# MaxInGaussian/SCFGP

Hardware: AMD Instinct MI355X
Metric: NLML+grad evals/sec (higher is better)
Workload: dtype f32

## Files before the change

scfgp_amd/csrc/kernels_kstage.hip:

```cpp
#include "kernels.h"
#include "tile_engine.h"

#ifndef SCFGP_KSTAGE_BK
#define SCFGP_KSTAGE_BK 16
#endif
#ifndef SCFGP_KSTAGE_WGM
#define SCFGP_KSTAGE_WGM 2
#define SCFGP_KSTAGE_WGN 2
#endif
typedef TileCfg<double, 64, 64, SCFGP_KSTAGE_BK, SCFGP_KSTAGE_WGM, SCFGP_KSTAGE_WGN> KCfg;
#define SMEM_DECL extern __shared__ __attribute__((aligned(16))) char smem_raw[]

struct GemmArgs {
    const double* A; const double* B; double* C;
    int64_t lda, ldb, ldc;
    int M, N, K;
    double alpha, beta;
    int tri;
    int kskip;
};

template <bool TRA, bool TRB>
__device__ __forceinline__ void gemm64_body(const GemmArgs& a, int tm, int tn, double* smem) {
    typedef KCfg Cfg;
    if (tm * Cfg::BM >= a.M || tn * Cfg::BN >= a.N) return;
    if (a.tri && tn > tm) return;
    const int k0 = a.kskip == 1 ? (tm > tn ? tm : tn) * Cfg::BM : (a.kskip == 2 ? tn * Cfg::BN : (a.kskip == 4 ? tm * Cfg::BM : 0));
    const int k1 = a.kskip == 3 && (tm + 1) * Cfg::BM < a.K ? (tm + 1) * Cfg::BM : a.K;
    const int nkt = (k1 - k0) / Cfg::BK;
    v4d acc[Cfg::TM][Cfg::TN];
    acc_zero<Cfg>(acc);
    if (TRA) {
        TrLoader<double, double, Cfg::BM, Cfg::BK, Cfg::LDA, Cfg::THREADS, false, false, 3> la(a.A + (int64_t)tm * Cfg::BM * a.lda + k0, a.lda, threadIdx.x);
        if (TRB) {
            TrLoader<double, double, Cfg::BN, Cfg::BK, Cfg::LDB, Cfg::THREADS, false, false, 3> lb(a.B + (int64_t)tn * Cfg::BN * a.ldb + k0, a.ldb, threadIdx.x);
            tile_mainloop_deep3<Cfg>(la, lb, nkt, acc, smem);
        } else {
            NatLoader<double, double, Cfg::BN, Cfg::BK, Cfg::LDB, Cfg::THREADS, false, false, false, 3> lb(a.B + (int64_t)k0 * a.ldb + tn * Cfg::BN, a.ldb, threadIdx.x);
            tile_mainloop_deep3<Cfg>(la, lb, nkt, acc, smem);
        }
    } else {
        NatLoader<double, double, Cfg::BM, Cfg::BK, Cfg::LDA, Cfg::THREADS, false, false, false, 3> la(a.A + (int64_t)k0 * a.lda + tm * Cfg::BM, a.lda, threadIdx.x);
        if (TRB) {
            TrLoader<double, double, Cfg::BN, Cfg::BK, Cfg::LDB, Cfg::THREADS, false, false, 3> lb(a.B + (int64_t)tn * Cfg::BN * a.ldb + k0, a.ldb, threadIdx.x);
            tile_mainloop_deep3<Cfg>(la, lb, nkt, acc, smem);
        } else {
            NatLoader<double, double, Cfg::BN, Cfg::BK, Cfg::LDB, Cfg::THREADS, false, false, false, 3> lb(a.B + (int64_t)k0 * a.ldb + tn * Cfg::BN, a.ldb, threadIdx.x);
            tile_mainloop_deep3<Cfg>(la, lb, nkt, acc, smem);
        }
    }
    AccCoord<Cfg> co;
#pragma unroll
    for (int t1 = 0; t1 < Cfg::TM; ++t1)
#pragma unroll
        for (int r = 0; r < Cfg::MTr::NACC; ++r) {
            double* c = a.C + (int64_t)(tm * Cfg::BM + co.row(t1, r)) * a.ldc + tn * Cfg::BN;
#pragma unroll
            for (int t2 = 0; t2 < Cfg::TN; ++t2) {
                const double v = a.alpha * acc[t1][t2][r];
                c[co.col(t2)] = a.beta == 0.0 ? v : v + a.beta * c[co.col(t2)];
                if (a.tri == 2 && tm != tn) a.C[(int64_t)(tn * Cfg::BN + co.col(t2)) * a.ldc + tm * Cfg::BM + co.row(t1, r)] = v;
            }
        }
}

template <bool TRA, bool TRB>
__global__ __launch_bounds__(KCfg::THREADS) void gemm64_kernel(GemmArgs a) {
    SMEM_DECL;
    gemm64_body<TRA, TRB>(a, blockIdx.y, blockIdx.x, reinterpret_cast<double*>(smem_raw));
}

template <bool TRA, bool TRB>
static void gemm64(const GemmArgs& a, hipStream_t st) {
    if (a.M <= 0 || a.N <= 0) return;
    allow_big_lds(gemm64_kernel<TRA, TRB>, KCfg::LDS_BYTES);
    hipLaunchKernelGGL((gemm64_kernel<TRA, TRB>), dim3(a.N / KCfg::BN, a.M / KCfg::BM), dim3(KCfg::THREADS), KCfg::LDS_BYTES, st, a);
}

__device__ __forceinline__ double lane_bcast(double x, int lane) {
    const int lo = __builtin_amdgcn_readlane(__double2loint(x), lane), hi = __builtin_amdgcn_readlane(__double2hiint(x), lane);
    return __hiloint2double(hi, lo);
}
template <int NS>
__device__ __forceinline__ v4d mfma_tile(const double* pa, int lda, const double* pb, int ldbk, int ldbj, v4d acc, double sign) {
    const int lane = threadIdx.x & 63, i = lane & 15, q = lane >> 4;
#pragma unroll
    for (int s = 0; s < NS; ++s)
        acc = __builtin_amdgcn_mfma_f64_16x16x4f64(sign * pa[i * lda + 4 * s + q], pb[(4 * s + q) * ldbk + i * ldbj], acc, 0, 0, 0);
    return acc;
}
template <int LD>
__device__ __forceinline__ void block_xwt(const double* sX, const double* sW, v4d (&acc)[4]) {
    const int wave = threadIdx.x >> 6, lane = threadIdx.x & 63, i = lane & 15, q = lane >> 4;
#pragma unroll
    for (int b = 0; b < 4; ++b) acc[b] = v4d{0, 0, 0, 0};
#pragma unroll
    for (int s = 0; s < 16; ++s) {
        const double x = sX[(16 * wave + i) * LD + 4 * s + q];
#pragma unroll
        for (int b = s / 4; b < 4; ++b)
            acc[b] = __builtin_amdgcn_mfma_f64_16x16x4f64(x, sW[(16 * b + i) * LD + 4 * s + q], acc[b], 0, 0, 0);
    }
}
template <typename P>
__device__ __forceinline__ void block_store(P* dst, int64_t pitch, const v4d (&acc)[4]) {
    const int wave = threadIdx.x >> 6, lane = threadIdx.x & 63, ci = lane & 15, cq = lane >> 4;
#pragma unroll
    for (int b = 0; b < 4; ++b)
#pragma unroll
        for (int r = 0; r < 4; ++r) dst[(int64_t)(16 * wave + cq + 4 * r) * pitch + 16 * b + ci] = acc[b][r];
}
__device__ __forceinline__ void block_load(const double* src, int64_t pitch, v4d (&acc)[4]) {
    const int wave = threadIdx.x >> 6, lane = threadIdx.x & 63, ci = lane & 15, cq = lane >> 4;
#pragma unroll
    for (int b = 0; b < 4; ++b)
#pragma unroll
        for (int r = 0; r < 4; ++r) acc[b][r] = src[(int64_t)(16 * wave + cq + 4 * r) * pitch + 16 * b + ci];
}
template <int LD>
__device__ __forceinline__ void block_sub_pqt(const double* sP, const double* sQ, v4d (&acc)[4]) {
    const int wave = threadIdx.x >> 6, lane = threadIdx.x & 63, i = lane & 15, q = lane >> 4;
#pragma unroll
    for (int s = 0; s < 16; ++s) {
        const double x = -sP[(16 * wave + i) * LD + 4 * s + q];
#pragma unroll
        for (int b = 0; b < 4; ++b)
            acc[b] = __builtin_amdgcn_mfma_f64_16x16x4f64(x, sQ[(16 * b + i) * LD + 4 * s + q], acc[b], 0, 0, 0);
    }
}
template <int LD>
__device__ __forceinline__ void block_add_pqt(const double* sP, const double* sQ, v4d (&acc)[4]) {
    const int wave = threadIdx.x >> 6, lane = threadIdx.x & 63, i = lane & 15, q = lane >> 4;
#pragma unroll
    for (int s = 0; s < 16; ++s) {
        const double x = sP[(16 * wave + i) * LD + 4 * s + q];
#pragma unroll
        for (int b = 0; b < 4; ++b)
            acc[b] = __builtin_amdgcn_mfma_f64_16x16x4f64(x, sQ[(16 * b + i) * LD + 4 * s + q], acc[b], 0, 0, 0);
    }
}
__device__ __forceinline__ void block_to_lds(const double* src, int64_t pitch, double* dst, int LD) {
    for (int e = threadIdx.x; e < 64 * 64; e += 256) dst[(e / 64) * LD + e % 64] = src[(int64_t)(e / 64) * pitch + e % 64];
}

#ifdef SCFGP_TRACE
__device__ unsigned long long g_ctrace[64][16];
#define CSTAMP(k) do { if (threadIdx.x == 0 && p < 64) g_ctrace[p][k] = __builtin_amdgcn_s_memrealtime(); } while (0)
int64_t chol_trace_read(void* host, int64_t max_bytes) {
    const int64_t n = max_bytes < (int64_t)sizeof(g_ctrace) ? max_bytes : (int64_t)sizeof(g_ctrace);
    return hipMemcpyFromSymbol(host, HIP_SYMBOL(g_ctrace), n) == hipSuccess ? n : -2;
}
#else
#define CSTAMP(k)
int64_t chol_trace_read(void*, int64_t) { return -1; }
#endif

__global__ __launch_bounds__(256) void chol_step_kernel(double* A, double* Lm, double* Li, double* Bm, int64_t ld, int p, int nb, int* flag) {
    constexpr int NB = 64, LD = NB + 1, PB = 16;
    __shared__ double sL[NB * LD];
    __shared__ double sI[NB * LD];
    __shared__ double sT[32 * 33];
    __shared__ double sD[NB];
    const int tid = threadIdx.x, lane = tid & 63, wave = tid >> 6;
    const int ci = lane & 15, cq = lane >> 4;
    v4d acc[4];
    if (blockIdx.x > 0) {
        const int q = p - 1, n = nb - p, T = n * (n + 1) / 2, U = p * n;
        int t = blockIdx.x - 1, i, j;
        bool b_tile = false;
        const auto tri_decode = [](int t, int& ti, int& tj) {
            ti = (int)((sqrtf(8.0f * t + 1.0f) - 1.0f) * 0.5f);
            while ((ti + 1) * (ti + 2) / 2 <= t) ++ti;
            while (ti * (ti + 1) / 2 > t) --ti;
            tj = t - ti * (ti + 1) / 2;
        };
        if (t < T) {
            int ti, tj; tri_decode(t, ti, tj);
            i = p + ti; j = p + tj;
            if (i == p && j == p) return;
        } else if (t < T + U) {
            t -= T; i = t / n; j = p + t % n;
        } else {
            tri_decode(t - T - U, i, j); b_tile = true;
        }
        const double* gw = Li + ((int64_t)q * ld + q) * NB;
        const double* gi = A + ((int64_t)i * ld + q) * NB;
        const double* gj = A + ((int64_t)j * ld + q) * NB;
        double* c = (b_tile ? Bm : A) + ((int64_t)i * ld + j) * NB;
        const bool unit_i = i == q, unit_j = j == q;
        const bool first_b = b_tile && i == q;
        v2d rw[8], ri[8], rj[8];
#pragma unroll
        for (int u = 0; u < 8; ++u) {
            const int e = (tid + u * 256) * 2;
            const int64_t o = (int64_t)(e / NB) * ld + e % NB;
            rw[u] = *reinterpret_cast<const v2d*>(gw + o);
            if (!unit_i) ri[u] = *reinterpret_cast<const v2d*>(gi + o);
            if (i != j && !unit_j) rj[u] = *reinterpret_cast<const v2d*>(gj + o);
        }
        v4d accc[4];
        if (!first_b) block_load(c, ld, accc);
        else {
#pragma unroll
            for (int b = 0; b < 4; ++b) accc[b] = v4d{0, 0, 0, 0};
        }
#pragma unroll
        for (int u = 0; u < 8; ++u) {
            const int e = (tid + u * 256) * 2, o = (e / NB) * LD + e % NB;
            sL[o] = rw[u][0]; sL[o + 1] = rw[u][1];
            if (!unit_i) { sI[o] = ri[u][0]; sI[o + 1] = ri[u][1]; }
        }
        __syncthreads();
        const auto w_transposed = [&](v4d (&a)[4]) {
#pragma unroll
            for (int b = 0; b < 4; ++b)
#pragma unroll
                for (int r = 0; r < 4; ++r) a[b][r] = sL[(16 * b + ci) * LD + 16 * wave + cq + 4 * r];
        };
        if (unit_i) w_transposed(acc);
        else block_xwt<LD>(sI, sL, acc);
        v4d accj[4];
        if (i != j) {
            if (unit_j) w_transposed(accj);
            else {
                __syncthreads();
#pragma unroll
                for (int u = 0; u < 8; ++u) {
                    const int e = (tid + u * 256) * 2, o = (e / NB) * LD + e % NB;
                    sI[o] = rj[u][0]; sI[o + 1] = rj[u][1];
                }
                __syncthreads();
                block_xwt<LD>(sI, sL, accj);
            }
            if (b_tile && unit_i) {
                double* d = Li + ((int64_t)q * ld + j) * NB;
#pragma unroll
                for (int b = 0; b < 4; ++b)
#pragma unroll
                    for (int r = 0; r < 4; ++r) d[(int64_t)(16 * b + ci) * ld + 16 * wave + cq + 4 * r] = accj[b][r];
            }
        }
        __syncthreads();
        block_store(sL, LD, acc);
        if (i != j) block_store(sI, LD, accj);
        __syncthreads();
        if (b_tile) {
            block_add_pqt<LD>(sL, i != j ? sI : sL, accc);
            block_store(c, ld, accc);
            if (i != j) {
                double* ct = Bm + ((int64_t)j * ld + i) * NB;
#pragma unroll
                for (int b = 0; b < 4; ++b)
#pragma unroll
                    for (int r = 0; r < 4; ++r) ct[(int64_t)(16 * b + ci) * ld + 16 * wave + cq + 4 * r] = accc[b][r];
            }
            return;
        }
        block_sub_pqt<LD>(sL, i != j ? sI : sL, accc);
        block_store(c, ld, accc);
        return;
    }
    if (p >= nb) return;
    CSTAMP(0);
    double* a = A + ((int64_t)p * ld + p) * NB;
    if (p > 0) {
        const double* gx = A + ((int64_t)p * ld + (p - 1)) * NB;
        const double* gw = Li + ((int64_t)(p - 1) * ld + (p - 1)) * NB;
        v2d rx[8], rw[8];
#pragma unroll
        for (int i = 0; i < 8; ++i) {
            const int e = (tid + i * 256) * 2;
            rx[i] = *reinterpret_cast<const v2d*>(gx + (int64_t)(e / NB) * ld + e % NB);
            rw[i] = *reinterpret_cast<const v2d*>(gw + (int64_t)(e / NB) * ld + e % NB);
        }
        v4d accd[4];
        block_load(a, ld, accd);
#pragma unroll
        for (int i = 0; i < 8; ++i) {
            const int e = (tid + i * 256) * 2, o = (e / NB) * LD + e % NB;
            sI[o] = rx[i][0]; sI[o + 1] = rx[i][1];
            sL[o] = rw[i][0]; sL[o + 1] = rw[i][1];
        }
        __syncthreads();
        CSTAMP(12);
        block_xwt<LD>(sI, sL, acc);
        __syncthreads();
        block_store(sI, LD, acc);
        __syncthreads();
        CSTAMP(13);
#pragma unroll
        for (int b = 0; b < 4; ++b) acc[b] = accd[b];
        CSTAMP(14);
        block_sub_pqt<LD>(sI, sI, acc);
        __syncthreads();
        CSTAMP(15);
        block_store(sL, LD, acc);
        for (int e = tid; e < NB * NB; e += 256) sI[(e / NB) * LD + e % NB] = 0.0;
    } else {
        for (int e = tid; e < NB * NB; e += 256) {
            sL[(e / NB) * LD + e % NB] = a[(int64_t)(e / NB) * ld + e % NB];
            sI[(e / NB) * LD + e % NB] = 0.0;
        }
    }
    double* lm = Lm + ((int64_t)p * ld + p) * NB;
    double* li = Li + ((int64_t)p * ld + p) * NB;
    bool bad = false;
    CSTAMP(1);
    const auto tile_update = [&](int r0, int c0, int pp) {
        v4d acc;
#pragma unroll
        for (int r = 0; r < 4; ++r) acc[r] = sL[(r0 + cq + 4 * r) * LD + c0 + ci];
        acc = mfma_tile<4>(sL + r0 * LD + pp, LD, sL + c0 * LD + pp, 1, LD, acc, -1.0);
#pragma unroll
        for (int r = 0; r < 4; ++r) sL[(r0 + cq + 4 * r) * LD + c0 + ci] = acc[r];
    };
    for (int pb = 0; pb < NB; pb += PB) {
        __syncthreads();
        const int nt = (NB - pb) / PB;
        if (wave == 0) {
            if (pb > 0)
                for (int ti = 0; ti < nt; ++ti) tile_update(pb + PB * ti, pb, pb - PB);
            const int row = pb + lane;
            double v[PB], invs[PB];
#pragma unroll
            for (int c = 0; c < PB; ++c) v[c] = row < NB ? sL[row * LD + pb + c] : 0.0;
#pragma unroll
            for (int j = 0; j < PB; ++j) {
                const double d = lane_bcast(v[j], j);
                bad |= !(d > 0.0);
                double inv = __builtin_amdgcn_rsq(d);
                inv = fma(0.5 * inv, fma(-d * inv, inv, 1.0), inv);
                inv = fma(0.5 * inv, fma(-d * inv, inv, 1.0), inv);
                invs[j] = inv;
                v[j] *= inv;
#pragma unroll
                for (int k = j + 1; k < PB; ++k) v[k] = fma(-v[j], lane_bcast(v[j], k), v[k]);
            }
#pragma unroll
            for (int c = 0; c < PB; ++c)
                if (row < NB) sL[row * LD + pb + c] = v[c];
            if (lane == 0) {
#pragma unroll
                for (int c = 0; c < PB; ++c) sD[pb + c] = invs[c];
            }
            CSTAMP(2 + pb / PB * 2);
            CSTAMP(3 + pb / PB * 2);
        } else if (pb > 0) {
            int t = 0;
            for (int tj = 1; tj < nt; ++tj)
                for (int ti = tj; ti < nt; ++ti, ++t)
                    if (t % 3 == wave - 1) tile_update(pb + PB * ti, pb + PB * tj, pb - PB);
        }
    }
    if (bad && tid == 0) *flag = 1;
    __syncthreads();
    if (tid < NB) {
        const int o = (tid / PB) * PB, c = tid % PB;
        double sres[PB];
#pragma unroll
        for (int r = 0; r < PB; ++r) sres[r] = r == c ? 1.0 : 0.0;
#pragma unroll
        for (int k = 0; k < PB; ++k) {
            const double xk = k >= c ? sres[k] * sD[o + k] : 0.0;
            sI[(o + k) * LD + o + c] = xk;
#pragma unroll
            for (int r = k + 1; r < PB; ++r) sres[r] = fma(-sL[(o + r) * LD + o + k], xk, sres[r]);
        }
    }
    __syncthreads();
    CSTAMP(10);
    for (int h = PB; h < NB; h *= 2) {
        const int npair = NB / (2 * h), tpp = (h / PB) * (h / PB), LT = h + 1;
        for (int t = wave; t < npair * tpp; t += 4) {
            const int q = t / tpp, ti = (t % tpp) / (h / PB), tj = t % (h / PB), o = q * 2 * h;
            v4d acc = {0, 0, 0, 0};
            acc = h == PB ? mfma_tile<4>(sL + (o + h + PB * ti) * LD + o, LD, sI + o * LD + o + PB * tj, LD, 1, acc, 1.0)
                          : mfma_tile<8>(sL + (o + h + PB * ti) * LD + o, LD, sI + o * LD + o + PB * tj, LD, 1, acc, 1.0);
#pragma unroll
            for (int r = 0; r < 4; ++r) sT[q * 16 * 17 + (PB * ti + cq + 4 * r) * LT + PB * tj + ci] = acc[r];
        }
        __syncthreads();
        for (int t = wave; t < npair * tpp; t += 4) {
            const int q = t / tpp, ti = (t % tpp) / (h / PB), tj = t % (h / PB), o = q * 2 * h;
            v4d acc = {0, 0, 0, 0};
            acc = h == PB ? mfma_tile<4>(sI + (o + h + PB * ti) * LD + o + h, LD, sT + q * 16 * 17 + PB * tj, LT, 1, acc, -1.0)
                          : mfma_tile<8>(sI + (o + h + PB * ti) * LD + o + h, LD, sT + q * 16 * 17 + PB * tj, LT, 1, acc, -1.0);
#pragma unroll
            for (int r = 0; r < 4; ++r) sI[(o + h + PB * ti + cq + 4 * r) * LD + o + PB * tj + ci] = acc[r];
        }
        __syncthreads();
    }
    for (int e = tid; e < NB * NB; e += 256) {
        const int i = e / NB, k = e % NB;
        lm[(int64_t)i * ld + k] = k <= i ? sL[i * LD + k] : 0.0;
        li[(int64_t)i * ld + k] = sI[i * LD + k];
    }
    CSTAMP(11);
}

__global__ __launch_bounds__(256) void kstage_unpack_kernel(const double* __restrict__ packed, int B, double* __restrict__ A, double* __restrict__ Li,
                                                            double* __restrict__ Bm, int64_t ld, int K, int nbk, const Scal* __restrict__ sc) {
    const int t = blockIdx.x;
    int ti = (int)((sqrtf(8.0f * t + 1.0f) - 1.0f) * 0.5f);
    while ((ti + 1) * (ti + 2) / 2 <= t) ++ti;
    while (ti * (ti + 1) / 2 > t) --ti;
    const int tj = t - ti * (ti + 1) / 2;
    const double lam = sc->lam;
    for (int e = blockIdx.y * 256 + threadIdx.x; e < B * B; e += gridDim.y * 256) {
        const double v = packed[(int64_t)t * B * B + e];
        const int i = ti * B + e / B, j = tj * B + e % B;
        A[(int64_t)i * ld + j] = j / 64 > i / 64 ? 0.0 : (i == j ? v + (i < K ? lam : 1.0) : v);
        if (ti != tj) A[(int64_t)j * ld + i] = 0.0;
        if (i / 64 >= nbk || j / 64 >= nbk) {
            const double id = i == j ? 1.0 : 0.0;
            Li[(int64_t)i * ld + j] = id; Bm[(int64_t)i * ld + j] = id;
            if (ti != tj) { Li[(int64_t)j * ld + i] = 0.0; Bm[(int64_t)j * ld + i] = 0.0; }
        }
    }
}

__global__ __launch_bounds__(256) void gemv_rows_kernel(const double* __restrict__ M, int64_t ld, const double* __restrict__ v,
                                                        double* __restrict__ out, int n) {
    const int lane = threadIdx.x & 63;
    const int i = blockIdx.x * 4 + (threadIdx.x >> 6);
    if (i >= n) return;
    double s = 0;
    for (int k = lane; k < n; k += 64) s += M[(int64_t)i * ld + k] * v[k];
#pragma unroll
    for (int m = 32; m >= 1; m >>= 1) s += __shfl_xor(s, m);
    if (lane == 0) out[i] = s;
}
__global__ __launch_bounds__(256) void factor_scalars_kernel(const double* __restrict__ L, const double* __restrict__ B, int64_t ld, int K,
                                                             const double* __restrict__ g, const double* __restrict__ alpha,
                                                             double* __restrict__ scalars) {
    __shared__ double r1[256], r2[256], r3[256], r4[256], r5[256];
    double s1 = 0, s2 = 0, lmin = 1.0 / 0.0, lmax = 0, bmax = 0;
    for (int i = threadIdx.x; i < K; i += 256) {
        const double l = L[(int64_t)i * ld + i], b = B[(int64_t)i * ld + i];
        s1 += log(l); s2 += g[i] * alpha[i];
        lmin = fmin(lmin, l * l); lmax = fmax(lmax, l * l); bmax = fmax(bmax, b);
    }
    r1[threadIdx.x] = s1; r2[threadIdx.x] = s2; r3[threadIdx.x] = lmin; r4[threadIdx.x] = lmax; r5[threadIdx.x] = bmax;
    __syncthreads();
    for (int m = 128; m >= 1; m >>= 1) {
        if (threadIdx.x < m) {
            r1[threadIdx.x] += r1[threadIdx.x + m]; r2[threadIdx.x] += r2[threadIdx.x + m];
            r3[threadIdx.x] = fmin(r3[threadIdx.x], r3[threadIdx.x + m]);
            r4[threadIdx.x] = fmax(r4[threadIdx.x], r4[threadIdx.x + m]);
            r5[threadIdx.x] = fmax(r5[threadIdx.x], r5[threadIdx.x + m]);
        }
        __syncthreads();
    }
    if (threadIdx.x == 0) {
        scalars[R_LOGDET] = 2.0 * r1[0]; scalars[R_GTALPHA] = r2[0];
        scalars[R_LMIN2] = r3[0]; scalars[R_LMAX2] = r4[0]; scalars[R_BMAX] = r5[0];
    }
}

__global__ __launch_bounds__(256) void abar_kernel(const double* __restrict__ B, const double* __restrict__ BWB, double* __restrict__ Abar,
                                                   const double* __restrict__ u, const double* __restrict__ al, int Kp,
                                                   const Scal* __restrict__ sc) {
    const double em2a = sc->em2a;
    const int64_t total = (int64_t)Kp * Kp;
    for (int64_t e = (int64_t)blockIdx.x * 256 + threadIdx.x; e < total; e += (int64_t)gridDim.x * 256) {
        const int i = (int)(e / Kp), j = (int)(e % Kp);
        Abar[e] = B[e] - BWB[e] - 0.5 * (u[i] * al[j] + al[i] * u[j]) + em2a * al[i] * al[j];
    }
}
__global__ __launch_bounds__(256) void adjoint_vec_kernel(const double* __restrict__ Abar, int64_t ld, int K, int Kp,
                                                          const double* __restrict__ u, const double* __restrict__ al,
                                                          double* __restrict__ ut, const Scal* __restrict__ sc,
                                                          double* __restrict__ scalars) {
    __shared__ double r1[256];
    const double em2a = sc->em2a;
    double s = 0;
    for (int i = threadIdx.x; i < Kp; i += 256) {
        ut[i] = u[i] - 2.0 * em2a * al[i];
        if (i < K) s += Abar[(int64_t)i * ld + i];
    }
    r1[threadIdx.x] = s;
    __syncthreads();
    for (int m = 128; m >= 1; m >>= 1) {
        if (threadIdx.x < m) r1[threadIdx.x] += r1[threadIdx.x + m];
        __syncthreads();
    }
    if (threadIdx.x == 0) scalars[R_TRABAR] = r1[0];
}

__global__ __launch_bounds__(256) void trace_ag_kernel(const double* __restrict__ packed, const double* __restrict__ Abar, int64_t ld,
                                                       int K, double* __restrict__ part) {
    constexpr int B = 128;
    __shared__ double r1[256];
    const int t = blockIdx.x;
    int ti = (int)((sqrtf(8.0f * t + 1.0f) - 1.0f) * 0.5f);
    while ((ti + 1) * (ti + 2) / 2 <= t) ++ti;
    while (ti * (ti + 1) / 2 > t) --ti;
    const int tj = t - ti * (ti + 1) / 2;
    double s = 0;
    for (int e = threadIdx.x; e < B * B; e += 256) {
        const int i = ti * B + e / B, j = tj * B + e % B;
        if (i < K && j < K) s += packed[(int64_t)t * B * B + e] * Abar[(int64_t)i * ld + j];
    }
    r1[threadIdx.x] = s;
    __syncthreads();
    for (int m = 128; m >= 1; m >>= 1) {
        if (threadIdx.x < m) r1[threadIdx.x] += r1[threadIdx.x + m];
        __syncthreads();
    }
    if (threadIdx.x == 0) part[t] = (ti == tj ? 1.0 : 2.0) * r1[0];
}
__global__ __launch_bounds__(256) void bbar_sums_kernel(const double* __restrict__ part, int ntiles, const double* __restrict__ ut,
                                                        const double* __restrict__ g, int K, double* __restrict__ scalars) {
    __shared__ double r1[256], r2[256];
    double s = 0, d = 0;
    for (int t = threadIdx.x; t < ntiles; t += 256) s += part[t];
    for (int i = threadIdx.x; i < K; i += 256) d += ut[i] * g[i];
    r1[threadIdx.x] = s; r2[threadIdx.x] = d;
    __syncthreads();
    for (int m = 128; m >= 1; m >>= 1) {
        if (threadIdx.x < m) { r1[threadIdx.x] += r1[threadIdx.x + m]; r2[threadIdx.x] += r2[threadIdx.x + m]; }
        __syncthreads();
    }
    if (threadIdx.x == 0) { scalars[R_TRAG] = r1[0]; scalars[R_UTG] = r2[0]; }
}
void kstage_bbar(const KStage& k, const double* packed, const double* Abar, double* part, hipStream_t st) {
    const int nts = k.Kp / 128, ntiles = nts * (nts + 1) / 2;
    hipLaunchKernelGGL(trace_ag_kernel, dim3(ntiles), dim3(256), 0, st, packed, Abar, (int64_t)k.Kp, k.K, part);
    hipLaunchKernelGGL(bbar_sums_kernel, dim3(1), dim3(256), 0, st, part, ntiles, k.ut, k.g, k.K, k.scalars);
}

static void cholesky_inverse_gram(const KStage& k, hipStream_t st) {
    const int nbk = (k.K + 63) / 64;
    for (int p = 0; p <= nbk; ++p) {
        const int n = nbk - p, items = p > 0 ? n * (n + 1) / 2 + p * n + p * (p + 1) / 2 : 0;
        hipLaunchKernelGGL(chol_step_kernel, dim3(1 + items), dim3(256), 0, st, k.A, k.T2, k.Li, k.B, (int64_t)k.Kp, p, nbk, k.flag);
    }
}

void kstage_factor(const KStage& k, const double* packed, const Scal* sc, hipStream_t st) {
    const int Kp = k.Kp, nts = Kp / 128, nbk = (k.K + 63) / 64;
    const int64_t ld = Kp;
    hipLaunchKernelGGL(kstage_unpack_kernel, dim3(nts * (nts + 1) / 2, 16), dim3(256), 0, st, packed, 128, k.A, k.Li, k.B, ld, k.K, nbk, sc);
    cholesky_inverse_gram(k, st);
    hipLaunchKernelGGL(gemv_rows_kernel, dim3((Kp + 3) / 4), dim3(256), 0, st, k.B, ld, k.g, k.alpha, Kp);
    hipLaunchKernelGGL(gemv_rows_kernel, dim3((Kp + 3) / 4), dim3(256), 0, st, k.Li, ld, k.g, k.beta, Kp);
    hipLaunchKernelGGL(factor_scalars_kernel, dim3(1), dim3(256), 0, st, k.T2, k.B, ld, k.K, k.g, k.alpha, k.scalars);
}

__global__ __launch_bounds__(256) void gemv_cols_part_kernel(const double* __restrict__ M, int64_t ld, const double* __restrict__ v,
                                                             double* __restrict__ part, int n) {
    const int i = blockIdx.x * 256 + threadIdx.x;
    const int per = (n + gridDim.y - 1) / gridDim.y, k0 = blockIdx.y * per, k1 = k0 + per < n ? k0 + per : n;
    if (i >= n) return;
    double s = 0;
    for (int k = k0 > i ? k0 : i; k < k1; ++k) s += M[(int64_t)k * ld + i] * v[k];
    part[(int64_t)blockIdx.y * n + i] = s;
}
__global__ __launch_bounds__(256) void gemv_cols_sum_kernel(const double* __restrict__ part, int nparts, double* __restrict__ out, int n) {
    const int i = blockIdx.x * 256 + threadIdx.x;
    if (i >= n) return;
    double s = 0;
    for (int p = 0; p < nparts; ++p) s += part[(int64_t)p * n + i];
    out[i] = s;
}

void kstage_adjoint_factor_form(const KStage& k, double* McBWB, double* Abar, const Scal* sc, hipStream_t st) {
    const int Kp = k.Kp;
    const int64_t ld = Kp;
    GemmArgs a1 = {McBWB, k.Li, k.T1, ld, ld, ld, Kp, Kp, Kp, 1.0, 0.0, 0, 2};
    gemm64<false, false>(a1, st);
    GemmArgs a2 = {k.Li, k.T1, McBWB, ld, ld, ld, Kp, Kp, Kp, 1.0, 0.0, 2, 4};
    gemm64<false, false>(a2, st);
    constexpr int PARTS = 32;
    hipLaunchKernelGGL(gemv_cols_part_kernel, dim3((Kp + 255) / 256, PARTS), dim3(256), 0, st, k.Li, ld, k.h, k.T1, Kp);
    hipLaunchKernelGGL(gemv_cols_sum_kernel, dim3((Kp + 255) / 256), dim3(256), 0, st, k.T1, PARTS, k.u, Kp);
    hipLaunchKernelGGL(abar_kernel, dim3(1024), dim3(256), 0, st, k.B, McBWB, Abar, k.u, k.alpha, Kp, sc);
    hipLaunchKernelGGL(adjoint_vec_kernel, dim3(1), dim3(256), 0, st, Abar, ld, k.K, Kp, k.u, k.alpha, k.ut, sc, k.scalars);
}

void kstage_adjoint(const KStage& k, const double* BWB, double* Abar, const Scal* sc, hipStream_t st) {
    const int Kp = k.Kp;
    const int64_t ld = Kp;
    hipLaunchKernelGGL(abar_kernel, dim3(1024), dim3(256), 0, st, k.B, BWB, Abar, k.h, k.alpha, Kp, sc);
    hipLaunchKernelGGL(adjoint_vec_kernel, dim3(1), dim3(256), 0, st, Abar, ld, k.K, Kp, k.h, k.alpha, k.ut, sc, k.scalars);
}
```

Measured before the change: 4.975.

## Make Cholesky step tiles persistent with prefetch and register-resident operand fragments

Caps each chol_step launch at the number of co-resident workgroups and gives each workgroup a contiguous range of update tiles. The shared W tile is staged in LDS once per workgroup, and the next tile's operands are prefetched into registers while the current tile computes. Operand panels go straight into per-lane register fragments instead of through LDS, and the MFMA loops skip blocks that are known to be zero (triangular). The trivial diagonal item is dropped from the grid and launch bounds now request two workgroups per CU. In exchange the kernel uses more registers and carries more complex indexing, and work can become imbalanced when the item count is just above the resident cap.

```diff
diff --git a/scfgp_amd/csrc/kernels_kstage.hip b/scfgp_amd/csrc/kernels_kstage.hip
--- a/scfgp_amd/csrc/kernels_kstage.hip
+++ b/scfgp_amd/csrc/kernels_kstage.hip
@@ -128,17 +128,6 @@
             acc[b] = __builtin_amdgcn_mfma_f64_16x16x4f64(x, sQ[(16 * b + i) * LD + 4 * s + q], acc[b], 0, 0, 0);
     }
 }
-template <int LD>
-__device__ __forceinline__ void block_add_pqt(const double* sP, const double* sQ, v4d (&acc)[4]) {
-    const int wave = threadIdx.x >> 6, lane = threadIdx.x & 63, i = lane & 15, q = lane >> 4;
-#pragma unroll
-    for (int s = 0; s < 16; ++s) {
-        const double x = sP[(16 * wave + i) * LD + 4 * s + q];
-#pragma unroll
-        for (int b = 0; b < 4; ++b)
-            acc[b] = __builtin_amdgcn_mfma_f64_16x16x4f64(x, sQ[(16 * b + i) * LD + 4 * s + q], acc[b], 0, 0, 0);
-    }
-}
 __device__ __forceinline__ void block_to_lds(const double* src, int64_t pitch, double* dst, int LD) {
     for (int e = threadIdx.x; e < 64 * 64; e += 256) dst[(e / 64) * LD + e % 64] = src[(int64_t)(e / 64) * pitch + e % 64];
 }
@@ -155,7 +144,7 @@
 int64_t chol_trace_read(void*, int64_t) { return -1; }
 #endif
 
-__global__ __launch_bounds__(256) void chol_step_kernel(double* A, double* Lm, double* Li, double* Bm, int64_t ld, int p, int nb, int* flag) {
+__global__ __launch_bounds__(256, 2) void chol_step_kernel(double* A, double* Lm, double* Li, double* Bm, int64_t ld, int p, int nb, int* flag) {
     constexpr int NB = 64, LD = NB + 1, PB = 16;
     __shared__ double sL[NB * LD];
     __shared__ double sI[NB * LD];
@@ -165,99 +154,124 @@
     const int ci = lane & 15, cq = lane >> 4;
     v4d acc[4];
     if (blockIdx.x > 0) {
-        const int q = p - 1, n = nb - p, T = n * (n + 1) / 2, U = p * n;
-        int t = blockIdx.x - 1, i, j;
-        bool b_tile = false;
+        const int q = p - 1, n = nb - p, T = n * (n + 1) / 2, U = p * n, skip = n > 0 ? 1 : 0;
+        const int items = T + U + p * (p + 1) / 2 - skip, nwg = gridDim.x - 1;
+        const int t0 = (int)((int64_t)items * (blockIdx.x - 1) / nwg), t1 = (int)((int64_t)items * blockIdx.x / nwg);
+        if (t0 >= t1) return;
         const auto tri_decode = [](int t, int& ti, int& tj) {
             ti = (int)((sqrtf(8.0f * t + 1.0f) - 1.0f) * 0.5f);
             while ((ti + 1) * (ti + 2) / 2 <= t) ++ti;
             while (ti * (ti + 1) / 2 > t) --ti;
             tj = t - ti * (ti + 1) / 2;
         };
-        if (t < T) {
-            int ti, tj; tri_decode(t, ti, tj);
-            i = p + ti; j = p + tj;
-            if (i == p && j == p) return;
-        } else if (t < T + U) {
-            t -= T; i = t / n; j = p + t % n;
-        } else {
-            tri_decode(t - T - U, i, j); b_tile = true;
-        }
+        const auto decode = [&](int t, int& i, int& j, bool& b_tile) {
+            t += skip; b_tile = false;
+            if (t < T) { int ti, tj; tri_decode(t, ti, tj); i = p + ti; j = p + tj; }
+            else if (t < T + U) { t -= T; i = t / n; j = p + t % n; }
+            else { tri_decode(t - T - U, i, j); b_tile = true; }
+        };
+        const auto load_frag = [&](const double* g, double (&x)[16]) {
+            const double* r = g + (int64_t)(16 * wave + ci) * ld + cq;
+#pragma unroll
+            for (int s = 0; s < 16; ++s) x[s] = r[4 * s];
+        };
+        const auto request = [&](int i, int j, bool b_tile, double (&xi)[16], double (&xj)[16], v4d (&cc)[4]) {
+            if (i != q) load_frag(A + ((int64_t)i * ld + q) * NB, xi);
+            if (i != j) load_frag(A + ((int64_t)j * ld + q) * NB, xj);
+            if (!(b_tile && i == q)) block_load((b_tile ? Bm : A) + ((int64_t)i * ld + j) * NB, ld, cc);
+            else {
+#pragma unroll
+                for (int b = 0; b < 4; ++b) cc[b] = v4d{0, 0, 0, 0};
+            }
+        };
         const double* gw = Li + ((int64_t)q * ld + q) * NB;
-        const double* gi = A + ((int64_t)i * ld + q) * NB;
-        const double* gj = A + ((int64_t)j * ld + q) * NB;
-        double* c = (b_tile ? Bm : A) + ((int64_t)i * ld + j) * NB;
-        const bool unit_i = i == q, unit_j = j == q;
-        const bool first_b = b_tile && i == q;
-        v2d rw[8], ri[8], rj[8];
+        v2d rw[8];
 #pragma unroll
         for (int u = 0; u < 8; ++u) {
             const int e = (tid + u * 256) * 2;
-            const int64_t o = (int64_t)(e / NB) * ld + e % NB;
-            rw[u] = *reinterpret_cast<const v2d*>(gw + o);
-            if (!unit_i) ri[u] = *reinterpret_cast<const v2d*>(gi + o);
-            if (i != j && !unit_j) rj[u] = *reinterpret_cast<const v2d*>(gj + o);
-        }
+            rw[u] = *reinterpret_cast<const v2d*>(gw + (int64_t)(e / NB) * ld + e % NB);
+        }
+        int i, j;
+        bool b_tile;
+        double xi[16], xj[16];
         v4d accc[4];
-        if (!first_b) block_load(c, ld, accc);
-        else {
-#pragma unroll
-            for (int b = 0; b < 4; ++b) accc[b] = v4d{0, 0, 0, 0};
-        }
+        decode(t0, i, j, b_tile);
+        request(i, j, b_tile, xi, xj, accc);
 #pragma unroll
         for (int u = 0; u < 8; ++u) {
             const int e = (tid + u * 256) * 2, o = (e / NB) * LD + e % NB;
             sL[o] = rw[u][0]; sL[o + 1] = rw[u][1];
-            if (!unit_i) { sI[o] = ri[u][0]; sI[o + 1] = ri[u][1]; }
-        }
-        __syncthreads();
-        const auto w_transposed = [&](v4d (&a)[4]) {
-#pragma unroll
-            for (int b = 0; b < 4; ++b)
-#pragma unroll
-                for (int r = 0; r < 4; ++r) a[b][r] = sL[(16 * b + ci) * LD + 16 * wave + cq + 4 * r];
-        };
-        if (unit_i) w_transposed(acc);
-        else block_xwt<LD>(sI, sL, acc);
-        v4d accj[4];
-        if (i != j) {
-            if (unit_j) w_transposed(accj);
-            else {
-                __syncthreads();
-#pragma unroll
-                for (int u = 0; u < 8; ++u) {
-                    const int e = (tid + u * 256) * 2, o = (e / NB) * LD + e % NB;
-                    sI[o] = rj[u][0]; sI[o + 1] = rj[u][1];
+        }
+        __syncthreads();
+        for (int t = t0; t < t1; ++t) {
+            const bool unit_i = i == q, diag = i == j;
+            if (unit_i) {
+#pragma unroll
+                for (int b = 0; b < 4; ++b)
+#pragma unroll
+                    for (int r = 0; r < 4; ++r) acc[b][r] = sL[(16 * b + cq + 4 * r) * LD + 16 * wave + ci];
+            } else {
+#pragma unroll
+                for (int b = 0; b < 4; ++b) acc[b] = v4d{0, 0, 0, 0};
+#pragma unroll
+                for (int s = 0; s < 16; ++s)
+#pragma unroll
+                    for (int b = s / 4; b < 4; ++b)
+                        acc[b] = __builtin_amdgcn_mfma_f64_16x16x4f64(sL[(16 * b + ci) * LD + 4 * s + cq], xi[s], acc[b], 0, 0, 0);
+            }
+            v4d accj[4];
+            if (!diag) {
+#pragma unroll
+                for (int b = 0; b < 4; ++b) accj[b] = v4d{0, 0, 0, 0};
+#pragma unroll
+                for (int s = 0; s < 16; ++s)
+#pragma unroll
+                    for (int b = s / 4; b < 4; ++b)
+                        accj[b] = __builtin_amdgcn_mfma_f64_16x16x4f64(xj[s], sL[(16 * b + ci) * LD + 4 * s + cq], accj[b], 0, 0, 0);
+                if (b_tile && unit_i) {
+                    double* d = Li + ((int64_t)q * ld + j) * NB;
+#pragma unroll
+                    for (int b = 0; b < 4; ++b)
+#pragma unroll
+                        for (int r = 0; r < 4; ++r) d[(int64_t)(16 * b + ci) * ld + 16 * wave + cq + 4 * r] = accj[b][r];
                 }
-                __syncthreads();
-                block_xwt<LD>(sI, sL, accj);
-            }
-            if (b_tile && unit_i) {
-                double* d = Li + ((int64_t)q * ld + j) * NB;
+            }
+            double* c = (b_tile ? Bm : A) + ((int64_t)i * ld + j) * NB;
+            double* ct = b_tile && !diag ? Bm + ((int64_t)j * ld + i) * NB : nullptr;
+            const double sign = b_tile ? 1.0 : -1.0;
+            const bool q_is_wt = unit_i && diag;
+            v4d accn[4];
+            if (t + 1 < t1) { decode(t + 1, i, j, b_tile); request(i, j, b_tile, xi, xj, accn); }
+            __syncthreads();
+            if (!diag) block_store(sI, LD, accj);
+            else if (!q_is_wt) {
 #pragma unroll
                 for (int b = 0; b < 4; ++b)
 #pragma unroll
-                    for (int r = 0; r < 4; ++r) d[(int64_t)(16 * b + ci) * ld + 16 * wave + cq + 4 * r] = accj[b][r];
-            }
-        }
-        __syncthreads();
-        block_store(sL, LD, acc);
-        if (i != j) block_store(sI, LD, accj);
-        __syncthreads();
-        if (b_tile) {
-            block_add_pqt<LD>(sL, i != j ? sI : sL, accc);
+                    for (int r = 0; r < 4; ++r) sI[(16 * wave + ci) * LD + 16 * b + cq + 4 * r] = acc[b][r];
+            }
+            __syncthreads();
+            const double* sQ = q_is_wt ? sL : sI;
+            const int qr = q_is_wt ? 1 : LD, qk = q_is_wt ? LD : 1;
+#pragma unroll
+            for (int s = 0; s < 16; ++s) {
+                const double x = sign * acc[s / 4][s % 4];
+#pragma unroll
+                for (int b = 0; b < 4; ++b)
+                    accc[b] = __builtin_amdgcn_mfma_f64_16x16x4f64(x, sQ[(16 * b + ci) * qr + (4 * s + cq) * qk], accc[b], 0, 0, 0);
+            }
             block_store(c, ld, accc);
-            if (i != j) {
-                double* ct = Bm + ((int64_t)j * ld + i) * NB;
+            if (ct) {
 #pragma unroll
                 for (int b = 0; b < 4; ++b)
 #pragma unroll
                     for (int r = 0; r < 4; ++r) ct[(int64_t)(16 * b + ci) * ld + 16 * wave + cq + 4 * r] = accc[b][r];
             }
-            return;
-        }
-        block_sub_pqt<LD>(sL, i != j ? sI : sL, accc);
-        block_store(c, ld, accc);
+            if (t + 1 < t1) {
+#pragma unroll
+                for (int b = 0; b < 4; ++b) accc[b] = accn[b];
+            }
+        }
         return;
     }
     if (p >= nb) return;
@@ -529,11 +543,22 @@
     hipLaunchKernelGGL(bbar_sums_kernel, dim3(1), dim3(256), 0, st, part, ntiles, k.ut, k.g, k.K, k.scalars);
 }
 
+static int chol_resident() {
+    static int n = 0;
+    if (n) return n;
+    int dev = 0, cus = 0, per = 0;
+    if (hipGetDevice(&dev) == hipSuccess && hipDeviceGetAttribute(&cus, hipDeviceAttributeMultiprocessorCount, dev) == hipSuccess &&
+        hipOccupancyMaxActiveBlocksPerMultiprocessor(&per, chol_step_kernel, 256, 0) == hipSuccess && cus > 0 && per > 0) n = cus * per;
+    else n = 512;
+    return n;
+}
 static void cholesky_inverse_gram(const KStage& k, hipStream_t st) {
     const int nbk = (k.K + 63) / 64;
+    const int room = chol_resident() - 1;
     for (int p = 0; p <= nbk; ++p) {
-        const int n = nbk - p, items = p > 0 ? n * (n + 1) / 2 + p * n + p * (p + 1) / 2 : 0;
-        hipLaunchKernelGGL(chol_step_kernel, dim3(1 + items), dim3(256), 0, st, k.A, k.T2, k.Li, k.B, (int64_t)k.Kp, p, nbk, k.flag);
+        const int n = nbk - p, items = p > 0 ? n * (n + 1) / 2 + p * n + p * (p + 1) / 2 - (n > 0 ? 1 : 0) : 0;
+        const int per = (items + room - 1) / room, nwg = per > 1 ? (items + per - 1) / per : items;
+        hipLaunchKernelGGL(chol_step_kernel, dim3(1 + nwg), dim3(256), 0, st, k.A, k.T2, k.Li, k.B, (int64_t)k.Kp, p, nbk, k.flag);
     }
 }
 
```

Measured after the change: 4.963. About the same (-0.2%).
